# indygreg/python-zstandard

Hardware: NVIDIA H100
Metric: uncompressed GB/s (compress+decompress) (higher is better)
Workload: dtype u8

## Files before the change

### python_zstandard_b200/csrc/zb_entropy.cuh

```cuda
#pragma once

#define ZB_ENT_WS_BYTES   256
#define ZB_ENT_WS_STRIDE  (ZB_ENT_WS_BYTES + 16)
#define ZB_ENT_SKEW(b)    ((((b) + 15u) & ~15u) | 16u)
#define ZB_ENT_DEF_LL     512
#define ZB_ENT_DEF_OF     (ZB_ENT_DEF_LL + 2 * 64)
#define ZB_ENT_DEF_ML     (ZB_ENT_DEF_OF + 2 * 32)
#define ZB_ENT_HEAD_BYTES (ZB_ENT_DEF_ML + 2 * 64)
#define ZB_ENT_POOL_BYTES(W) ((((227 * 1024 - ZB_ENT_HEAD_BYTES) / (W))) & ~15)
#define ZB_ENT_SMEM(W)    ((W) * ZB_ENT_POOL_BYTES(W) + ZB_ENT_HEAD_BYTES)

enum : u32 { ZB_SRC_NONE = 0, ZB_SRC_PREDEF = 1, ZB_SRC_RLE = 2, ZB_SRC_NCOUNT = 3, ZB_SRC_DICT = 4 };
struct ZbTabSrc { u32 kind; u32 sym; const u8* p; u32 n; };

enum : u32 { ZB_BD_FIRST = 1, ZB_BD_FSE_VALID = 2, ZB_BD_SKIP = 4 };
struct ZbBlkDesc {
    u64 hdr_off;
    u64 seq_off, lit_off;
    u32 span;
    u32 frame;
    u32 flags;
    u32 block_max;
    ZbTabSrc dHuf, dLL, dOF, dML;
};
struct ZbBlkExit { u32 rep[3]; u32 err; };

__device__ __forceinline__ u32 zb_warp_incl_scan(u32 v, u32 lane)
{
    #pragma unroll
    for (int d = 1; d < 32; d <<= 1) { u32 y = __shfl_up_sync(0xFFFFFFFFu, v, d); if (lane >= (u32)d) v += y; }
    return v;
}

template <int WORDS, int BITS>
struct ZbPacked {
    static constexpr u32 PER = 32 / BITS, MASK = (1u << BITS) - 1;
    u32 w[WORDS];
    __device__ __forceinline__ void clear() {
        #pragma unroll
        for (int j = 0; j < WORDS; j++) w[j] = 0;
    }
    __device__ __forceinline__ u32 get(u32 i) const {
        u32 const q = i / PER; u32 v = w[0];
        #pragma unroll
        for (int j = 1; j < WORDS; j++) v = q == (u32)j ? w[j] : v;
        return (v >> (BITS * (i - q * PER))) & MASK;
    }
    __device__ __forceinline__ void add(u32 i, u32 v) {
        u32 const q = i / PER, d = v << (BITS * (i - q * PER));
        #pragma unroll
        for (int j = 0; j < WORDS; j++) w[j] += q == (u32)j ? d : 0u;
    }
};
struct ZbRank : ZbPacked<4, 10> {
    __device__ __forceinline__ u32 operator[](u32 wt) const { return get(wt - 1); }
    __device__ __forceinline__ void count(u32 wt) { if (wt) add(wt - 1, 1); }
};

__device__ static u32 zb_huf_weights(u8* ws, const u8* s, u32 n, u32& out_log, u32& out_nsym, ZbRank& rank, ZB_RING_ARG(ring))
{
    u8* const wn = ws;
    u16* const wt = (u16*)(ws + 128);
    u32 nsym, hdr;
    if (n == 0) return 0;
    rank.clear();
    u32 total = 0;
    auto put = [&](u32 i, u32 w) { wn[i >> 1] |= (u8)(w << ((i & 1) * 4)); };
    auto clear_nibbles = [&] { for (int i = 0; i < 32; i++) ((u32*)wn)[i] = 0; };
    if (s[0] >= 128) {
        nsym = (u32)s[0] - 127; hdr = (nsym + 1) / 2;
        if (hdr + 1 > n) return 0;
        clear_nibbles();
        for (u32 i = 0; i < nsym; i++) {
            u32 b = s[1 + i / 2], w = (i & 1) ? (b & 15) : (b >> 4);
            if (w > 12) return 0;
            put(i, w); rank.count(w); total += (1u << w) >> 1;
        }
    } else {
        hdr = s[0];
        if (hdr + 1 > n) return 0;
        short* const norm = (short*)wn; u32 max_sym = 15, log;
        u32 const used = zb_read_ncount(norm, max_sym, log, s + 1, hdr);
        if (used == 0 || log > 6) return 0;
        zb_fse_spread(wt, norm, max_sym, log);
        u32 const size = 1u << log;
        for (u32 u = 0; u < size; u++) {
            u32 const sy = wt[u], x = (u32)(u16)norm[sy]; norm[sy] = (short)(x + 1);
            u32 const nb = log - (u32)zb_hibit(x);
            wt[u] = (u16)(sy | (nb << 4) | (((x << nb) - size) << 8));
        }
        clear_nibbles();
        ZbBitR<4> b;
        if (!b.init(s + 1 + used, hdr - used, ring)) return 0;
        u32 s1 = b.read(log), s2 = b.read(log); b.refill();
        if (b.left() < 0) return 0;
        nsym = 0;
        for (;;) {
            if (nsym + 2 > 255) return 0;
            { u32 c = wt[s1], w = c & 15; if (w > 12) return 0; put(nsym, w); rank.count(w); total += (1u << w) >> 1; nsym++;
              s1 = (c >> 8) + b.read((c >> 4) & 15); b.refill(); }
            if (b.left() < 0) { u32 w = wt[s2] & 15; if (w > 12) return 0; put(nsym, w); rank.count(w); total += (1u << w) >> 1; nsym++; break; }
            if (nsym + 2 > 255) return 0;
            { u32 c = wt[s2], w = c & 15; if (w > 12) return 0; put(nsym, w); rank.count(w); total += (1u << w) >> 1; nsym++;
              s2 = (c >> 8) + b.read((c >> 4) & 15); b.refill(); }
            if (b.left() < 0) { u32 w = wt[s1] & 15; if (w > 12) return 0; put(nsym, w); rank.count(w); total += (1u << w) >> 1; nsym++; break; }
        }
    }
    if (total == 0) return 0;
    u32 const log = (u32)zb_hibit(total) + 1;
    if (log > 12) return 0;
    u32 const rest = (1u << log) - total, hb = (u32)zb_hibit(rest);
    if ((1u << hb) != rest) return 0;
    put(nsym, hb + 1); rank.count(hb + 1); nsym++;
    if (rank[1] < 2 || (rank[1] & 1)) return 0;
    out_log = log; out_nsym = nsym;
    return hdr + 1;
}

#define ZB_HUF_COARSE 8u
struct ZbHufTab { const u16* cells; u32 log, shift, T, base; };
__device__ __forceinline__ void zb_huf_shape(u32 log, ZbRank const& rank, u32& shift, u32& T, u32& base, u32& bytes)
{
    shift = log > ZB_HUF_COARSE ? log - ZB_HUF_COARSE : 0u;
    T = 0;
    #pragma unroll
    for (u32 wt = 1; wt <= 12 - ZB_HUF_COARSE; wt++) T += wt <= shift ? rank[wt] << (wt - 1) : 0u;
    base = (T + 3u) & ~3u;
    bytes = 2u * (base + (1u << (log - shift)));
}
__device__ __forceinline__ ZbHufTab zb_huf_full(const u16* cells, u32 log) { ZbHufTab t; t.cells = cells; t.log = log; t.shift = 0; t.T = 0; t.base = 0; return t; }
#define ZB_HCELL(t, v) ((t).cells[(v) < (t).T ? (v) : (t).base + ((v) >> (t).shift)])

__device__ static void zb_huf_fill(u16* cells, const u8* ws, u32 log, u32 nsym, ZbRank const& rank, u32 shift, u32 base)
{
    ZbPacked<6, 16> next; next.clear();
    {
        u32 p = 0;
        #pragma unroll
        for (u32 wt = 1; wt <= 12; wt++) { next.add(wt - 1, p); p += wt <= log ? (rank[wt] << (wt - 1)) : 0; }
    }
    for (u32 i = 0; i < nsym; i++) {
        u32 const wt = (ws[i >> 1] >> ((i & 1) * 4)) & 15; if (!wt) continue;
        u32 len = 1u << (wt - 1), p = next.get(wt - 1); next.add(wt - 1, len);
        if (wt > shift) { len >>= shift; p = base + (p >> shift); }
        u32 const cell = i | ((log + 1 - wt) << 8);
        if (len >= 4) { u64 const v = cell * 0x0001000100010001ull; u64* q = (u64*)(cells + p); for (u32 k = 0; k < len / 4; k++) q[k] = v; }
        else if (len == 2) *(u32*)(cells + p) = cell * 0x00010001u;
        else cells[p] = (u16)cell;
    }
}

#ifdef ZB_SIMT_EMULATION
__device__ __forceinline__ ZbRank zb_rank_pack(const u32* rank) { ZbRank r; r.clear(); for (u32 wt = 1; wt <= 12; wt++) r.add(wt - 1, rank[wt]); return r; }
__device__ static u32 zb_huf_weights(u8* ws, const u8* s, u32 n, u32& out_log, u32& out_nsym, u32* rank, ZB_RING_ARG(ring))
{
    ZbRank r; u32 const used = zb_huf_weights(ws, s, n, out_log, out_nsym, r, ring);
    rank[0] = used ? out_nsym : 0;
    for (u32 w = 1; w <= 12; w++) { rank[w] = used ? r[w] : 0; rank[0] -= rank[w]; }
    return used;
}
__device__ __forceinline__ void zb_huf_shape(u32 log, const u32* rank, u32& shift, u32& T, u32& base, u32& bytes)
{
    zb_huf_shape(log, zb_rank_pack(rank), shift, T, base, bytes);
}
__device__ static void zb_huf_fill(u16* cells, const u8* ws, u32 log, u32 nsym, const u32* rank, u32 shift, u32 base)
{
    zb_huf_fill(cells, ws, log, nsym, zb_rank_pack(rank), shift, base);
}
#endif

__device__ static bool zb_huf_stream2(u8* out, u32 n_out, const u8* s, u32 n, ZbHufTab const t, u8* ring)
{
    ZbBitR<4> b;
    if (!b.init(s, n, ring)) return false;
    u32 const log = t.log;
    u32 i = 0;
    while (i < n_out && ((uintptr_t)(out + i) & 3)) { u32 v = b.peek(log); u32 c = ZB_HCELL(t, v); out[i++] = (u8)c; b.skip(c >> 8); b.refill(); }
    for (; i + 4 <= n_out; i += 4) {
        u32 v0 = b.peek(log); u32 c0 = ZB_HCELL(t, v0); b.skip(c0 >> 8);
        u32 v1 = b.peek(log); u32 c1 = ZB_HCELL(t, v1); b.skip(c1 >> 8); b.refill();
        u32 v2 = b.peek(log); u32 c2 = ZB_HCELL(t, v2); b.skip(c2 >> 8);
        u32 v3 = b.peek(log); u32 c3 = ZB_HCELL(t, v3); b.skip(c3 >> 8); b.refill();
        *(u32*)(out + i) = (c0 & 255) | ((c1 & 255) << 8) | ((c2 & 255) << 16) | (c3 << 24);
    }
    for (; i < n_out; i++) { u32 v = b.peek(log); u32 c = ZB_HCELL(t, v); out[i] = (u8)c; b.skip(c >> 8); b.refill(); }
    return b.left() == 0;
}

struct ZbHufLane { ZbBitR<4> b; u8* out; u32 left; };

__device__ __forceinline__ void zb_huf_one(ZbHufLane& h, ZbHufTab const& t)
{
    u32 const v = h.b.peek(t.log); u32 const c = ZB_HCELL(t, v); *h.out++ = (u8)c; h.b.skip(c >> 8); h.b.refill(); h.left--;
}
#define ZB_HUF4(h) do { \
        u32 const v0_ = h.b.peek(t.log); u32 const c0_ = ZB_HCELL(t, v0_); h.b.skip(c0_ >> 8); \
        u32 const v1_ = h.b.peek(t.log); u32 const c1_ = ZB_HCELL(t, v1_); h.b.skip(c1_ >> 8); h.b.refill(); \
        u32 const v2_ = h.b.peek(t.log); u32 const c2_ = ZB_HCELL(t, v2_); h.b.skip(c2_ >> 8); \
        u32 const v3_ = h.b.peek(t.log); u32 const c3_ = ZB_HCELL(t, v3_); h.b.skip(c3_ >> 8); h.b.refill(); \
        *(u32*)h.out = (c0_ & 255) | ((c1_ & 255) << 8) | ((c2_ & 255) << 16) | (c3_ << 24); h.out += 4; h.left -= 4; } while (0)

__device__ static bool zb_huf_block(u8* dstl, u32 regen, const u8* p, u32 left, bool single, ZbHufTab const t, ZB_RING_ARG(ring))
{
    if (single) return zb_huf_stream2(dstl, regen, p, left, t, ring);
    if (left < 10) return false;
    u32 const l1 = zb_rd16(p), l2 = zb_rd16(p + 2), l3 = zb_rd16(p + 4), seg = (regen + 3) / 4;
    if (6 + l1 + l2 + l3 > left || seg * 3 > regen) return false;
    u32 const l4 = left - 6 - l1 - l2 - l3;
    ZbHufLane h0, h1, h2, h3;
    u8* const r1 = ring ? ring + 64 : nullptr; u8* const r2 = ring ? ring + 128 : nullptr; u8* const r3 = ring ? ring + 192 : nullptr;
    if (!h0.b.start(p + 6, l1, ring) || !h1.b.start(p + 6 + l1, l2, r1) || !h2.b.start(p + 6 + l1 + l2, l3, r2) || !h3.b.start(p + 6 + l1 + l2 + l3, l4, r3)) return false;
    if (!h0.b.finish() || !h1.b.finish() || !h2.b.finish() || !h3.b.finish()) return false;
    h0.out = dstl; h1.out = dstl + seg; h2.out = dstl + 2 * seg; h3.out = dstl + 3 * seg;
    h0.left = h1.left = h2.left = seg; h3.left = regen - 3 * seg;
    while (h0.left && ((uintptr_t)h0.out & 3)) zb_huf_one(h0, t);
    while (h1.left && ((uintptr_t)h1.out & 3)) zb_huf_one(h1, t);
    while (h2.left && ((uintptr_t)h2.out & 3)) zb_huf_one(h2, t);
    while (h3.left && ((uintptr_t)h3.out & 3)) zb_huf_one(h3, t);
    while (h0.left >= 4 && h1.left >= 4 && h2.left >= 4 && h3.left >= 4) { ZB_HUF4(h0); ZB_HUF4(h1); ZB_HUF4(h2); ZB_HUF4(h3); }
    while (h0.left >= 4) ZB_HUF4(h0);
    while (h1.left >= 4) ZB_HUF4(h1);
    while (h2.left >= 4) ZB_HUF4(h2);
    while (h3.left >= 4) ZB_HUF4(h3);
    while (h0.left) zb_huf_one(h0, t);
    while (h1.left) zb_huf_one(h1, t);
    while (h2.left) zb_huf_one(h2, t);
    while (h3.left) zb_huf_one(h3, t);
    return h0.b.left() == 0 && h1.b.left() == 0 && h2.b.left() == 0 && h3.b.left() == 0;
}

__device__ static int zb_seq_desc(ZbTabSrc& d, u32 mode, u32 max_sym_kind, u32 max_log, const u8* ip, u32 avail,
                                  bool repeat_ok, short* norm, u32& log, u32& max_sym, u32& need)
{
    int used = 0;
    if (mode == 0) { d.kind = ZB_SRC_PREDEF; }
    else if (mode == 1) { if (avail == 0 || ip[0] > max_sym_kind) return -1; d.kind = ZB_SRC_RLE; d.sym = ip[0]; used = 1; }
    else if (mode == 2) { d.kind = ZB_SRC_NCOUNT; d.p = ip; d.n = avail; }
    else if (!repeat_ok || d.kind == ZB_SRC_NONE) return -1;
    need = 0; log = 0; max_sym = max_sym_kind;
    if (d.kind == ZB_SRC_NCOUNT) {
        u32 const u = zb_read_ncount(norm, max_sym, log, d.p, d.n);
        if (u == 0 || log > max_log) return -1;
        if (mode == 2) { used = (int)u; d.n = u; }
        need = 2u << log;
    } else if (d.kind == ZB_SRC_RLE) need = 2;
    return used;
}

template <class F> __device__ __forceinline__ void zb_cta_for(u32 n, F f)
{
#ifdef __CUDA_ARCH__
    for (u32 i = threadIdx.x; i < n; i += blockDim.x) f(i);
#else
    if (threadIdx.x == 0) for (u32 i = 0; i < n; i++) f(i);
#endif
}

__device__ __forceinline__ void zb_cta_cells16(u8* dst, const ZbFseCell* src, u32 log)
{
    zb_cta_for(1u << log, [&](u32 i) { u32 const c = src[i]; ((u16*)dst)[i] = ZB_CELL16(ZB_CELL_SYM(c), (ZB_CELL_NEXT(c) + (1u << log)) >> ZB_CELL_NB(c)); });
}

template <int W>
__device__ __forceinline__ u32 zb_ent_head(u8* smem, ZbDictDev const& dict)
{
    u32* const lutLL = (u32*)smem; u32* const lutML = lutLL + 36;
    zb_cta_for(36, [&](u32 i) { lutLL[i] = c_LL_base[i] | ((u32)c_LL_bits[i] << 24); });
    zb_cta_for(53, [&](u32 i) { lutML[i] = c_ML_base[i] | ((u32)c_ML_bits[i] << 24); });
    zb_cta_cells16(smem + ZB_ENT_DEF_LL, g_defLL, 6);
    zb_cta_cells16(smem + ZB_ENT_DEF_OF, g_defOF, 5);
    zb_cta_cells16(smem + ZB_ENT_DEF_ML, g_defML, 6);
    u32 head = ZB_ENT_HEAD_BYTES;
    if (dict.has_entropy) {
        zb_cta_cells16(smem + head, dict.ll, dict.ll_log); head += 2u << dict.ll_log;
        zb_cta_cells16(smem + head, dict.of, dict.of_log); head += 2u << dict.of_log;
        zb_cta_cells16(smem + head, dict.ml, dict.ml_log); head += 2u << dict.ml_log;
    }
    __syncthreads();
    return ((ZB_ENT_SMEM(W) - head) / W) & ~15u;
}

#ifdef ZB_PHASE_TIMERS
__device__ unsigned long long g_zb_ent_phase[8];
#define ZB_EMARK(k) do { if (lane == 0) { long long const t_ = clock64(); atomicAdd(&g_zb_ent_phase[k], (unsigned long long)(t_ - t_ph)); t_ph = t_; } } while (0)
#elif defined(ZB_DEBUG_BLOCKS)
#define ZB_EMARK(k) do { if (err && !(t_ph & 1)) { printf("[emark %d] lane %u err %u\n", k, lane, err); t_ph |= 1; } } while (0)
#else
#define ZB_EMARK(k) do { (void)t_ph; } while (0)
#endif

template <bool SYMREP>
__device__ __forceinline__ u32 zb_seq_block(const u8* smem, u8* q, u8* ws, ZbDictDev const& dict,
                                            ZbTabSrc const& dLL, ZbTabSrc const& dOF, ZbTabSrc const& dML,
                                            u32 msLL, u32 msOF, u32 msML, u32 logLL, u32 logOF, u32 logML,
                                            const u8* ip, const u8* bend, u32 nseq, ZbSeq* sq, u32 n_lit, u64 room, u64 hist,
                                            u32& rep0, u32& rep1, u32& rep2, u32& lit_used, u32& produced, long long& t_ph)
{
    const u32* const lutLL = (const u32*)smem; const u32* const lutML = lutLL + 36;
    short* const normLL = (short*)ws; short* const normOF = normLL + 36; short* const normML = normOF + 32;
    u32 const dct_ll = ZB_ENT_HEAD_BYTES, dct_of = dct_ll + (2u << dict.ll_log), dct_ml = dct_of + (2u << dict.of_log);
    ZbTab tLL, tOF, tML;
    auto setup = [&](const ZbTabSrc& d, short* norm, u32 ms, u32 lg, int kind, u32 dct, u32 dlog, u32 def, u32 deflog, ZbTab& t) {
        if (d.kind == ZB_SRC_NCOUNT) { zb_build_fse((u16*)q, norm, ms, lg, kind); t.off = (u32)(q - smem); t.log = lg; q += 2u << lg; }
        else if (d.kind == ZB_SRC_RLE) { *(u16*)q = ZB_CELL16(d.sym, 1u); t.off = (u32)(q - smem); t.log = 0; q += 2; }
        else if (d.kind == ZB_SRC_DICT) { t.off = dct; t.log = dlog; }
        else { t.off = def; t.log = deflog; }
    };
    setup(dLL, normLL, msLL, logLL, K_LL, dct_ll, dict.ll_log, ZB_ENT_DEF_LL, 6, tLL);
    setup(dOF, normOF, msOF, logOF, K_OF, dct_of, dict.of_log, ZB_ENT_DEF_OF, 5, tOF);
    setup(dML, normML, msML, logML, K_ML, dct_ml, dict.ml_log, ZB_ENT_DEF_ML, 6, tML);
#ifdef ZB_PHASE_TIMERS
    { u32 const lane = threadIdx.x & 31; ZB_EMARK(7); }
#endif

    ZbBitR<8> b;
    if (!b.init(ip, (u32)(bend - ip), ws)) return ZB_E_CORRUPTION;
    u32 sLL = b.read(tLL.log); u32 sOF = b.read(tOF.log); b.refill(); u32 sML = b.read(tML.log);
    const u8* const TL = smem + tLL.off; const u8* const TO = smem + tOF.off; const u8* const TM = smem + tML.off;
    u32 const kL = 31 - tLL.log, kO = 31 - tOF.log, kM = 31 - tML.log;
    u32 err = ZB_OK;
    for (u32 i = 0; i < nseq; i++) {
        u32 const cl = *(const u16*)(TL + 2 * sLL), co = *(const u16*)(TO + 2 * sOF), cm = *(const u16*)(TM + 2 * sML);
        b.refill();
        u32 const llc = cl & 63, ofc = co & 63, xl = cl >> 6, xo = co >> 6, xm = cm >> 6;
        u32 const nl = __clz(xl) - kL, nm = __clz(xm) - kM, no = __clz(xo) - kO;
        u32 const eL = lutLL[llc], eM = lutML[cm & 63];
        u32 const llb = eL >> 24, ab = (eM >> 24) + llb;
        u32 const sb = i + 1 < nseq ? nl + nm + no : 0;
        bool const slow = (int)(ofc + ab + sb) > b.avail;
        u32 const ob = b.read(ofc);
        u32 ll = eL & 0xFFFFFFu, ml = eM & 0xFFFFFFu, off;
        if (ofc > 1) {
            off = (1u << ofc) - 3 + ob;
            if (SYMREP && (off & 0x80000000u)) { err = ZB_E_CORRUPTION; break; }
            rep2 = rep1; rep1 = rep0; rep0 = off;
        } else {
            u32 const ll0 = (llc == 0);
            if (ofc == 0) {
                if (ll0) { off = rep1; rep1 = rep0; rep0 = off; } else off = rep0;
            } else {
                u32 const idx = 1 + ll0 + ob;
                u32 const r0m = SYMREP && (rep0 & 0x80000000u) ? rep0 + 1 : rep0 - 1;
                u32 tmp = idx == 1 ? rep1 : (idx == 2 ? rep2 : r0m);
                if (SYMREP && tmp == 0) { err = ZB_E_CORRUPTION; break; }
                if (tmp == 0) tmp = 0xFFFFFFFFu;
                if (idx != 1) rep2 = rep1;
                rep1 = rep0; rep0 = off = tmp;
            }
        }
        if (slow) b.refill();
        {
            u32 const both = b.read(ab);
            ml += both >> llb; ll += both & ((1u << llb) - 1);
        }
        if (slow) b.refill();
        {
            u32 const v = b.read(sb);
            sLL = (xl << nl) - (1u << tLL.log) + (v >> (nm + no));
            sML = (xm << nm) - (1u << tML.log) + ((v >> no) & ((1u << nm) - 1));
            sOF = (xo << no) - (1u << tOF.log) + (v & ((1u << no) - 1));
        }
        sq[i] = make_uint4(lit_used, produced, ml, off);
        if ((u64)produced + ll + ml > room) { err = ZB_E_DSTSIZE_TOO_SMALL; break; }
        if (ll > n_lit - lit_used) { err = ZB_E_CORRUPTION; break; }
        lit_used += ll; produced += ll;
        if ((u64)off > hist + produced) { err = ZB_E_CORRUPTION; break; }
        produced += ml;
    }
    if (!err && b.left() != 0) err = ZB_E_CORRUPTION;
    return err;
}

template <int ZB_ENT_WARPS>
__global__ void __launch_bounds__(ZB_ENT_WARPS * 32)
zb_entropy_decode(const u8* __restrict__ src, const ZbSegment* __restrict__ segs, u32 n_frames,
                  const ZbFramePlace* __restrict__ place, const u64* __restrict__ dst_sizes,
                  ZbBlock* __restrict__ blocks, ZbSeq* __restrict__ seqs, u8* __restrict__ lits,
                  u32* __restrict__ work_counter, ZbDictDev dict, u32* status, u64* __restrict__ out_sizes,
                  u32* __restrict__ ck_expect, u32 take)
{
    ZB_DYN_SMEM(zb_smem);
    u32 const lane = threadIdx.x & 31, warp = threadIdx.x >> 5;
    u32 const pool_bytes = zb_ent_head<ZB_ENT_WARPS>(zb_smem, dict);
    u8* const pool = zb_smem + ZB_ENT_SMEM(ZB_ENT_WARPS) - (ZB_ENT_WARPS - warp) * pool_bytes;
    u8* const ws = pool + lane * ZB_ENT_WS_STRIDE;
    u8* const tabs = pool + 32 * ZB_ENT_WS_STRIDE;
    u32 const TAB_BYTES = pool_bytes - 32 * ZB_ENT_WS_STRIDE;

    for (;;) {
        u32 base = 0;
        if (lane == 0) base = atomicAdd(work_counter, take);
        base = __shfl_sync(0xFFFFFFFFu, base, 0);
        if (base >= n_frames) return;
        u32 const f = base + lane;
        bool done = lane >= take || !(f < n_frames) || status[f] != ZB_OK;

        const u8* s = src; u64 n = 0; ZbHdr h; ZbFramePlace pl; u32 err = ZB_OK;
        u64 cap = 0, out_pos = 0, blk_i = 0, seq_i = 0, lit_i = 0, pos = 0; u32 block_max = 0;
        u32 rep0 = 1, rep1 = 4, rep2 = 8;
        ZbTabSrc dHuf = {ZB_SRC_NONE, 0, nullptr, 0}, dLL = dHuf, dOF = dHuf, dML = dHuf;
        bool fse_valid = false;
        if (!done) {
            s = src + segs[f].offset; n = segs[f].length;
            zb_skip_skippable(s, n);
            zb_parse_header(s, n, h);
            pl = place[f]; cap = pl.dst_cap; blk_i = pl.blk_off; seq_i = pl.seq_off; lit_i = pl.lit_off; pos = h.hdr_size;
            block_max = h.window < ZB_BLOCK_MAX ? (u32)h.window : ZB_BLOCK_MAX;
            if (dict.has_entropy) {
                dHuf.kind = dLL.kind = dOF.kind = dML.kind = ZB_SRC_DICT; fse_valid = true;
                rep0 = dict.rep[0]; rep1 = dict.rep[1]; rep2 = dict.rep[2];
            }
            if (h.dict_id && dict.dict_id && h.dict_id != dict.dict_id) { err = ZB_E_DICT_WRONG; done = true; }
        }
        u64 const hist_extra = dict.content_size;

        long long t_ph = clock64() & ~1ll;
        while (__any_sync(0xFFFFFFFFu, !done)) {
            ZB_EMARK(0);
            ZbBlock B; B.kind = 0; B.regen = 0; B.n_seq = 0; B.n_lit = 0; B.lit_kind = 0; B.lit_byte = 0; B.src_pos = 0; B.seq_pos = seq_i; B.out_pos = out_pos;
            bool comp = false, last = false;
            u32 bsize = 0; const u8* bs = nullptr; const u8* bend = nullptr; const u8* ip = nullptr;
            ZbLitHdr L; L.type = 0; L.regen = 0; L.hdr = 0; L.csize = 0; L.single = 0;
            if (!done) {
                do {
                    if (pos + 3 > n) { err = ZB_E_SRCSIZE_WRONG; break; }
                    u32 const bh = zb_rd24(s + pos); pos += 3;
                    last = bh & 1; u32 const type = (bh >> 1) & 3; bsize = bh >> 3; B.kind = type;
                    if (type == 3) { err = ZB_E_CORRUPTION; break; }
                    if (type == ZB_BLK_RLE) {
                        if (pos + 1 > n) { err = ZB_E_SRCSIZE_WRONG; break; }
                        if (bsize > block_max) { err = ZB_E_CORRUPTION; break; }
                        if (bsize > cap - out_pos) { err = ZB_E_DSTSIZE_TOO_SMALL; break; }
                        B.src_pos = (u64)(s + pos - src); B.regen = bsize; B.lit_byte = s[pos]; pos += 1;
                    } else if (type == ZB_BLK_RAW) {
                        if (pos + bsize > n) { err = ZB_E_SRCSIZE_WRONG; break; }
                        if (bsize > block_max) { err = ZB_E_CORRUPTION; break; }
                        if (bsize > cap - out_pos) { err = ZB_E_DSTSIZE_TOO_SMALL; break; }
                        B.src_pos = (u64)(s + pos - src); B.regen = bsize; pos += bsize;
                    } else {
                        if (pos + bsize > n || bsize > block_max) { err = ZB_E_SRCSIZE_WRONG; break; }
                        bs = s + pos; bend = bs + bsize;
                        err = zb_parse_lit_header(bs, bsize, L);
                        if (err) break;
                        if (L.regen > block_max) { err = ZB_E_CORRUPTION; break; }
                        B.n_lit = L.regen; comp = true;
                    }
                } while (0);
                if (err) { done = true; comp = false; }
            }
            ZB_EMARK(1);
            bool wantH = false; u32 hlog = 0, hns = 0; ZbRank rank; const u8* hp = nullptr; u32 hleft = 0;
            if (comp) {
                do {
                    if (L.type == 0) {
                        if (L.hdr + L.regen > bsize) { err = ZB_E_CORRUPTION; break; }
                        B.lit_kind = ZB_LIT_RAW; B.src_pos = (u64)(bs + L.hdr - src); ip = bs + L.hdr + L.regen;
                    } else if (L.type == 1) {
                        if (L.hdr + 1 > bsize) { err = ZB_E_CORRUPTION; break; }
                        B.lit_kind = ZB_LIT_RLE; B.lit_byte = bs[L.hdr]; ip = bs + L.hdr + 1;
                    } else {
                        if (L.type == 3 && dHuf.kind == ZB_SRC_NONE) { err = ZB_E_DICT_CORRUPTED; break; }
                        if (!L.single && L.regen < 6) { err = ZB_E_LITERALS_HEADER_WRONG; break; }
                        if (L.csize + L.hdr > bsize || L.regen == 0) { err = ZB_E_CORRUPTION; break; }
                        hp = bs + L.hdr; hleft = L.csize;
                        if (L.type == 2) { dHuf.kind = ZB_SRC_NCOUNT; dHuf.p = hp; dHuf.n = hleft; }
                        if (dHuf.kind == ZB_SRC_NCOUNT) {
                            u32 const used = zb_huf_weights(ws, dHuf.p, dHuf.n, hlog, hns, rank, tabs + lane * 80);
                            if (used == 0 || (L.type == 2 && used >= hleft)) { err = ZB_E_CORRUPTION; break; }
                            if (L.type == 2) { hp += used; hleft -= used; dHuf.n = used; }
                            wantH = true;
                        }
                        B.lit_kind = ZB_LIT_SCRATCH; B.src_pos = lit_i; ip = bs + L.hdr + L.csize;
                    }
                } while (0);
                if (err) { done = true; comp = false; wantH = false; }
            }
            if (comp && B.lit_kind == ZB_LIT_SCRATCH && dHuf.kind == ZB_SRC_DICT) {
                if (!zb_huf_block(lits + lit_i, L.regen, hp, hleft, L.single, zb_huf_full(dict.huf, dict.huf_log), ws)) { err = ZB_E_CORRUPTION; done = true; comp = false; }
            }
            ZB_EMARK(2);
            {
                bool pending = wantH;
                u32 hshift = 0, hT = 0, hbase = 0, hbytes = 0;
                if (wantH) zb_huf_shape(hlog, rank, hshift, hT, hbase, hbytes);
                while (__any_sync(0xFFFFFFFFu, pending)) {
                    u32 const need = pending ? hbytes : 0;
                    u32 const incl = zb_warp_incl_scan((need + 15) & ~15u, lane);
                    if (pending && incl <= TAB_BYTES) {
                        u16* cells = (u16*)(tabs + incl - ((need + 15) & ~15u));
                        zb_huf_fill(cells, ws, hlog, hns, rank, hshift, hbase);
                        ZB_EMARK(6);
                        ZbHufTab t; t.cells = cells; t.log = hlog; t.shift = hshift; t.T = hT; t.base = hbase;
                        if (!zb_huf_block(lits + lit_i, L.regen, hp, hleft, L.single, t, ws)) { err = ZB_E_CORRUPTION; done = true; comp = false; }
                        pending = false;
                    }
                    __syncwarp();
                }
            }
            ZB_EMARK(3);
            if (comp && B.lit_kind == ZB_LIT_SCRATCH) lit_i += (L.regen + 15) & ~15u;
            u32 nseq = 0, logLL = 0, logOF = 0, logML = 0, msLL = 0, msOF = 0, msML = 0, needS = 0;
            short* const normLL = (short*)ws; short* const normOF = normLL + 36; short* const normML = normOF + 32;
            if (comp) {
                do {
                    if (ip >= bend) { err = ZB_E_SRCSIZE_WRONG; break; }
                    nseq = *ip++;
                    if (nseq > 0x7F) {
                        if (nseq == 0xFF) { if (ip + 2 > bend) { err = ZB_E_SRCSIZE_WRONG; break; } nseq = zb_rd16(ip) + 0x7F00; ip += 2; }
                        else { if (ip >= bend) { err = ZB_E_SRCSIZE_WRONG; break; } nseq = ((nseq - 0x80) << 8) + *ip++; }
                    }
                    B.n_seq = nseq;
                    if (nseq == 0) { if (ip != bend) err = ZB_E_CORRUPTION; break; }
                    if (ip + 1 > bend) { err = ZB_E_SRCSIZE_WRONG; break; }
                    u32 const modes = *ip++;
                    if (modes & 3) { err = ZB_E_CORRUPTION; break; }
                    u32 nd; int r;
                    r = zb_seq_desc(dLL, modes >> 6, 35, 9, ip, (u32)(bend - ip), fse_valid, normLL, logLL, msLL, nd);
                    if (r < 0) { err = ZB_E_CORRUPTION; break; } ip += r; needS += nd;
                    r = zb_seq_desc(dOF, (modes >> 4) & 3, 31, 8, ip, (u32)(bend - ip), fse_valid, normOF, logOF, msOF, nd);
                    if (r < 0) { err = ZB_E_CORRUPTION; break; } ip += r; needS += nd;
                    r = zb_seq_desc(dML, (modes >> 2) & 3, 52, 9, ip, (u32)(bend - ip), fse_valid, normML, logML, msML, nd);
                    if (r < 0) { err = ZB_E_CORRUPTION; break; } ip += r; needS += nd;
                    fse_valid = true;
                } while (0);
                if (err) { done = true; comp = false; nseq = 0; }
            }
            ZB_EMARK(4);
            u32 lit_used = 0, produced = 0;
            {
                bool pending = comp && nseq > 0;
                while (__any_sync(0xFFFFFFFFu, pending)) {
                    u32 const need = pending ? ZB_ENT_SKEW(needS) : 0;
                    u32 const incl = zb_warp_incl_scan(need, lane);
                    if (pending && incl <= TAB_BYTES) {
                        err = zb_seq_block<false>(zb_smem, tabs + incl - need, ws, dict, dLL, dOF, dML, msLL, msOF, msML, logLL, logOF, logML,
                                                   ip, bend, nseq, seqs + seq_i, L.regen, cap - out_pos, out_pos + hist_extra,
                                                   rep0, rep1, rep2, lit_used, produced, t_ph);
                        if (err) { done = true; comp = false; }
                        pending = false;
                    }
                    __syncwarp();
                }
            }
            ZB_EMARK(5);
            if (!done) {
                if (comp) {
                    seqs[seq_i + nseq] = make_uint4(lit_used, produced, 0, 0);
                    seq_i += nseq + 1;
                    u32 const tail = L.regen - lit_used;
                    if ((u64)produced + tail > cap - out_pos) err = ZB_E_DSTSIZE_TOO_SMALL;
                    B.regen = produced + tail;
                    if (!err && B.regen > block_max) err = ZB_E_CORRUPTION;
                    pos += bsize;
                }
                if (!err) {
                    blocks[blk_i++] = B;
                    out_pos += B.regen;
                    if (last) {
                        if (h.content_size != ZB_CONTENT_UNKNOWN && out_pos != h.content_size) err = ZB_E_CORRUPTION;
                        else if (h.checksum && pos + 4 > n) err = ZB_E_CHECKSUM_WRONG;
                        else {
                            if (h.checksum) ck_expect[f] = zb_rd32(s + pos);
                            if (dst_sizes && out_pos != cap) err = ZB_E_SIZE_MISMATCH;
                        }
                        done = true;
                    }
                }
                if (err) done = true;
            }
        }
        if (lane < take && f < n_frames && status[f] == ZB_OK) {
            if (err) { status[f] = err; out_sizes[f] = err == ZB_E_SIZE_MISMATCH ? out_pos : 0; } else out_sizes[f] = out_pos;
        } else if (lane < take && f < n_frames) out_sizes[f] = 0;
    }
}

template <int ZB_ENT_WARPS>
__global__ void __launch_bounds__(ZB_ENT_WARPS * 32)
zb_entropy_blocks(const u8* __restrict__ src, const ZbBlkDesc* __restrict__ bdesc, u32 n_blocks,
                  ZbBlock* __restrict__ blocks, ZbSeq* __restrict__ seqs, u8* __restrict__ lits,
                  u32* __restrict__ work_counter, ZbDictDev dict, u32* status, ZbBlkExit* __restrict__ bexit, u32 take)
{
    ZB_DYN_SMEM(zb_smem);
    u32 const lane = threadIdx.x & 31, warp = threadIdx.x >> 5;
    u32 const pool_bytes = zb_ent_head<ZB_ENT_WARPS>(zb_smem, dict);
    u8* const pool = zb_smem + ZB_ENT_SMEM(ZB_ENT_WARPS) - (ZB_ENT_WARPS - warp) * pool_bytes;
    u8* const ws = pool + lane * ZB_ENT_WS_BYTES;
    u8* const tabs = pool + 32 * ZB_ENT_WS_BYTES;
    u32 const TAB_BYTES = pool_bytes - 32 * ZB_ENT_WS_BYTES;

    for (;;) {
        u32 base = 0;
        if (lane == 0) base = atomicAdd(work_counter, take);
        base = __shfl_sync(0xFFFFFFFFu, base, 0);
        if (base >= n_blocks) return;
        u32 const bi = base + lane;
        ZbBlkDesc D; D.frame = 0; D.flags = 0;
        if (lane < take && bi < n_blocks) D = bdesc[bi];
        bool done = lane >= take || !(bi < n_blocks) || (D.flags & ZB_BD_SKIP) || status[D.frame] != ZB_OK;

        const u8* s = src; u64 n = 0; u32 err = ZB_OK;
        u64 const cap = ~0ull >> 1; u64 out_pos = 0, blk_i = bi, seq_i = 0, lit_i = 0, pos = 0; u32 block_max = 0;
        u32 rep0 = 1, rep1 = 4, rep2 = 8;
        ZbTabSrc dHuf = {ZB_SRC_NONE, 0, nullptr, 0}, dLL = dHuf, dOF = dHuf, dML = dHuf;
        bool fse_valid = false;
        if (!done) {
            s = src + D.hdr_off; n = D.span; seq_i = D.seq_off; lit_i = D.lit_off; block_max = D.block_max;
            dHuf = D.dHuf; dLL = D.dLL; dOF = D.dOF; dML = D.dML; fse_valid = (D.flags & ZB_BD_FSE_VALID) != 0;
            if (D.flags & ZB_BD_FIRST) { if (dict.has_entropy) { rep0 = dict.rep[0]; rep1 = dict.rep[1]; rep2 = dict.rep[2]; } }
            else { rep0 = 0x80000000u; rep1 = 0xA0000000u; rep2 = 0xC0000000u; }
        }
        u64 const hist_extra = 1ull << 40;

        long long t_ph = clock64() & ~1ll;
        while (__any_sync(0xFFFFFFFFu, !done)) {
            ZB_EMARK(0);
            ZbBlock B; B.kind = 0; B.regen = 0; B.n_seq = 0; B.n_lit = 0; B.lit_kind = 0; B.lit_byte = 0; B.src_pos = 0; B.seq_pos = seq_i; B.out_pos = out_pos;
            bool comp = false, last = false;
            u32 bsize = 0; const u8* bs = nullptr; const u8* bend = nullptr; const u8* ip = nullptr;
            ZbLitHdr L; L.type = 0; L.regen = 0; L.hdr = 0; L.csize = 0; L.single = 0;
            if (!done) {
                do {
                    if (pos + 3 > n) { err = ZB_E_SRCSIZE_WRONG; break; }
                    u32 const bh = zb_rd24(s + pos); pos += 3;
                    last = bh & 1; u32 const type = (bh >> 1) & 3; bsize = bh >> 3; B.kind = type;
                    if (type == 3) { err = ZB_E_CORRUPTION; break; }
                    if (type == ZB_BLK_RLE) {
                        if (pos + 1 > n) { err = ZB_E_SRCSIZE_WRONG; break; }
                        if (bsize > block_max) { err = ZB_E_CORRUPTION; break; }
                        if (bsize > cap - out_pos) { err = ZB_E_DSTSIZE_TOO_SMALL; break; }
                        B.src_pos = (u64)(s + pos - src); B.regen = bsize; B.lit_byte = s[pos]; pos += 1;
                    } else if (type == ZB_BLK_RAW) {
                        if (pos + bsize > n) { err = ZB_E_SRCSIZE_WRONG; break; }
                        if (bsize > block_max) { err = ZB_E_CORRUPTION; break; }
                        if (bsize > cap - out_pos) { err = ZB_E_DSTSIZE_TOO_SMALL; break; }
                        B.src_pos = (u64)(s + pos - src); B.regen = bsize; pos += bsize;
                    } else {
                        if (pos + bsize > n || bsize > block_max) { err = ZB_E_SRCSIZE_WRONG; break; }
                        bs = s + pos; bend = bs + bsize;
                        err = zb_parse_lit_header(bs, bsize, L);
                        if (err) break;
                        if (L.regen > block_max) { err = ZB_E_CORRUPTION; break; }
                        B.n_lit = L.regen; comp = true;
                    }
                } while (0);
                if (err) { done = true; comp = false; }
            }
            ZB_EMARK(1);
            bool wantH = false; u32 hlog = 0, hns = 0; ZbRank rank; const u8* hp = nullptr; u32 hleft = 0;
            if (comp) {
                do {
                    if (L.type == 0) {
                        if (L.hdr + L.regen > bsize) { err = ZB_E_CORRUPTION; break; }
                        B.lit_kind = ZB_LIT_RAW; B.src_pos = (u64)(bs + L.hdr - src); ip = bs + L.hdr + L.regen;
                    } else if (L.type == 1) {
                        if (L.hdr + 1 > bsize) { err = ZB_E_CORRUPTION; break; }
                        B.lit_kind = ZB_LIT_RLE; B.lit_byte = bs[L.hdr]; ip = bs + L.hdr + 1;
                    } else {
                        if (L.type == 3 && dHuf.kind == ZB_SRC_NONE) { err = ZB_E_DICT_CORRUPTED; break; }
                        if (!L.single && L.regen < 6) { err = ZB_E_LITERALS_HEADER_WRONG; break; }
                        if (L.csize + L.hdr > bsize || L.regen == 0) { err = ZB_E_CORRUPTION; break; }
                        hp = bs + L.hdr; hleft = L.csize;
                        if (L.type == 2) { dHuf.kind = ZB_SRC_NCOUNT; dHuf.p = hp; dHuf.n = hleft; }
                        if (dHuf.kind == ZB_SRC_NCOUNT) {
                            u32 const used = zb_huf_weights(ws, dHuf.p, dHuf.n, hlog, hns, rank, tabs + lane * 64);
                            if (used == 0 || (L.type == 2 && used >= hleft)) { err = ZB_E_CORRUPTION; break; }
                            if (L.type == 2) { hp += used; hleft -= used; dHuf.n = used; }
                            wantH = true;
                        }
                        B.lit_kind = ZB_LIT_SCRATCH; B.src_pos = lit_i; ip = bs + L.hdr + L.csize;
                    }
                } while (0);
                if (err) { done = true; comp = false; wantH = false; }
            }
            if (comp && B.lit_kind == ZB_LIT_SCRATCH && dHuf.kind == ZB_SRC_DICT) {
                if (!zb_huf_block(lits + lit_i, L.regen, hp, hleft, L.single, zb_huf_full(dict.huf, dict.huf_log), ws)) { err = ZB_E_CORRUPTION; done = true; comp = false; }
            }
            ZB_EMARK(2);
            {
                bool pending = wantH;
                u32 hshift = 0, hT = 0, hbase = 0, hbytes = 0;
                if (wantH) zb_huf_shape(hlog, rank, hshift, hT, hbase, hbytes);
                while (__any_sync(0xFFFFFFFFu, pending)) {
                    u32 const need = pending ? hbytes : 0;
                    u32 const incl = zb_warp_incl_scan((need + 15) & ~15u, lane);
                    if (pending && incl <= TAB_BYTES) {
                        u16* cells = (u16*)(tabs + incl - ((need + 15) & ~15u));
                        zb_huf_fill(cells, ws, hlog, hns, rank, hshift, hbase);
                        ZB_EMARK(6);
                        ZbHufTab t; t.cells = cells; t.log = hlog; t.shift = hshift; t.T = hT; t.base = hbase;
                        if (!zb_huf_block(lits + lit_i, L.regen, hp, hleft, L.single, t, ws)) { err = ZB_E_CORRUPTION; done = true; comp = false; }
                        pending = false;
                    }
                    __syncwarp();
                }
            }
            ZB_EMARK(3);
            if (comp && B.lit_kind == ZB_LIT_SCRATCH) lit_i += (L.regen + 15) & ~15u;
            u32 nseq = 0, logLL = 0, logOF = 0, logML = 0, msLL = 0, msOF = 0, msML = 0, needS = 0;
            short* const normLL = (short*)ws; short* const normOF = normLL + 36; short* const normML = normOF + 32;
            if (comp) {
                do {
                    if (ip >= bend) { err = ZB_E_SRCSIZE_WRONG; break; }
                    nseq = *ip++;
                    if (nseq > 0x7F) {
                        if (nseq == 0xFF) { if (ip + 2 > bend) { err = ZB_E_SRCSIZE_WRONG; break; } nseq = zb_rd16(ip) + 0x7F00; ip += 2; }
                        else { if (ip >= bend) { err = ZB_E_SRCSIZE_WRONG; break; } nseq = ((nseq - 0x80) << 8) + *ip++; }
                    }
                    B.n_seq = nseq;
                    if (nseq == 0) { if (ip != bend) err = ZB_E_CORRUPTION; break; }
                    if (ip + 1 > bend) { err = ZB_E_SRCSIZE_WRONG; break; }
                    u32 const modes = *ip++;
                    if (modes & 3) { err = ZB_E_CORRUPTION; break; }
                    u32 nd; int r;
                    r = zb_seq_desc(dLL, modes >> 6, 35, 9, ip, (u32)(bend - ip), fse_valid, normLL, logLL, msLL, nd);
                    if (r < 0) { err = ZB_E_CORRUPTION; break; } ip += r; needS += nd;
                    r = zb_seq_desc(dOF, (modes >> 4) & 3, 31, 8, ip, (u32)(bend - ip), fse_valid, normOF, logOF, msOF, nd);
                    if (r < 0) { err = ZB_E_CORRUPTION; break; } ip += r; needS += nd;
                    r = zb_seq_desc(dML, (modes >> 2) & 3, 52, 9, ip, (u32)(bend - ip), fse_valid, normML, logML, msML, nd);
                    if (r < 0) { err = ZB_E_CORRUPTION; break; } ip += r; needS += nd;
                    fse_valid = true;
                } while (0);
                if (err) { done = true; comp = false; nseq = 0; }
            }
            ZB_EMARK(4);
            u32 lit_used = 0, produced = 0;
            {
                bool pending = comp && nseq > 0;
                while (__any_sync(0xFFFFFFFFu, pending)) {
                    u32 const need = pending ? ((needS + 15) & ~15u) : 0;
                    u32 const incl = zb_warp_incl_scan(need, lane);
                    if (pending && incl <= TAB_BYTES) {
                        err = zb_seq_block<true>(zb_smem, tabs + incl - need, ws, dict, dLL, dOF, dML, msLL, msOF, msML, logLL, logOF, logML,
                                                   ip, bend, nseq, seqs + seq_i, L.regen, cap - out_pos, out_pos + hist_extra,
                                                   rep0, rep1, rep2, lit_used, produced, t_ph);
                        if (err) { done = true; comp = false; }
                        pending = false;
                    }
                    __syncwarp();
                }
            }
            ZB_EMARK(5);
            if (!done) {
                if (comp) {
                    seqs[seq_i + nseq] = make_uint4(lit_used, produced, 0, 0);
                    seq_i += nseq + 1;
                    u32 const tail = L.regen - lit_used;
                    if ((u64)produced + tail > cap - out_pos) err = ZB_E_DSTSIZE_TOO_SMALL;
                    B.regen = produced + tail;
                    if (!err && B.regen > block_max) err = ZB_E_CORRUPTION;
                    pos += bsize;
                }
                if (!err) blocks[blk_i] = B;
                done = true;
            }
        }
        if (lane < take && bi < n_blocks && !(D.flags & ZB_BD_SKIP)) {
            ZbBlkExit X; X.rep[0] = rep0; X.rep[1] = rep1; X.rep[2] = rep2; X.err = err;
            bexit[bi] = X;
#ifdef ZB_DEBUG_BLOCKS
            if (err) printf("[entropy_blocks] block %u frame %u err %u flags %u span %u | huf k%u n%u | LL k%u n%u s%u | OF k%u n%u s%u | ML k%u n%u s%u | hdr %02x %02x %02x | LLp-src %lld\n", bi, D.frame, err, D.flags, D.span,
                            D.dHuf.kind, D.dHuf.n, D.dLL.kind, D.dLL.n, D.dLL.sym, D.dOF.kind, D.dOF.n, D.dOF.sym, D.dML.kind, D.dML.n, D.dML.sym,
                            src[D.hdr_off], src[D.hdr_off + 1], src[D.hdr_off + 2], D.dLL.p ? (long long)(D.dLL.p - src) : -1ll);
#endif
            if (err) atomicCAS(&status[D.frame], (u32)ZB_OK, err);
        }
    }
}
```

Before: 147.9.

## Stage decoded sequences in shared memory and write them out warp-cooperatively

The per-lane sequence decode loop now writes each decoded sequence to a per-lane shared-memory staging ring of eight entries instead of storing it directly to global memory. Every eight sequences the warp synchronizes, and lanes cooperatively copy the staged entries to global memory, with eight lanes covering each source lane's batch, so that scattered 16-byte global stores become coalesced 128-byte bursts. The function is now called by all lanes, with a go flag, so that warp-collective shuffles work. In exchange it adds warp synchronization every eight sequences, which forces divergent lanes to wait on one another, and uses part of the workspace as staging with a stride that differs between the two call sites.

```diff
diff --git a/python_zstandard_b200/csrc/zb_entropy.cuh b/python_zstandard_b200/csrc/zb_entropy.cuh
--- a/python_zstandard_b200/csrc/zb_entropy.cuh
+++ b/python_zstandard_b200/csrc/zb_entropy.cuh
@@ -290,84 +290,109 @@
 #endif
 
 template <bool SYMREP>
-__device__ __forceinline__ u32 zb_seq_block(const u8* smem, u8* q, u8* ws, ZbDictDev const& dict,
+__device__ __forceinline__ u32 zb_seq_block(bool go, const u8* smem, u8* q, u8* ws, u32 ws_stride, ZbDictDev const& dict,
                                             ZbTabSrc const& dLL, ZbTabSrc const& dOF, ZbTabSrc const& dML,
                                             u32 msLL, u32 msOF, u32 msML, u32 logLL, u32 logOF, u32 logML,
                                             const u8* ip, const u8* bend, u32 nseq, ZbSeq* sq, u32 n_lit, u64 room, u64 hist,
                                             u32& rep0, u32& rep1, u32& rep2, u32& lit_used, u32& produced, long long& t_ph)
 {
+    u32 const lane = threadIdx.x & 31;
     const u32* const lutLL = (const u32*)smem; const u32* const lutML = lutLL + 36;
     short* const normLL = (short*)ws; short* const normOF = normLL + 36; short* const normML = normOF + 32;
     u32 const dct_ll = ZB_ENT_HEAD_BYTES, dct_of = dct_ll + (2u << dict.ll_log), dct_ml = dct_of + (2u << dict.of_log);
-    ZbTab tLL, tOF, tML;
+    ZbTab tLL = {0, 0}, tOF = tLL, tML = tLL;
     auto setup = [&](const ZbTabSrc& d, short* norm, u32 ms, u32 lg, int kind, u32 dct, u32 dlog, u32 def, u32 deflog, ZbTab& t) {
         if (d.kind == ZB_SRC_NCOUNT) { zb_build_fse((u16*)q, norm, ms, lg, kind); t.off = (u32)(q - smem); t.log = lg; q += 2u << lg; }
         else if (d.kind == ZB_SRC_RLE) { *(u16*)q = ZB_CELL16(d.sym, 1u); t.off = (u32)(q - smem); t.log = 0; q += 2; }
         else if (d.kind == ZB_SRC_DICT) { t.off = dct; t.log = dlog; }
         else { t.off = def; t.log = deflog; }
     };
-    setup(dLL, normLL, msLL, logLL, K_LL, dct_ll, dict.ll_log, ZB_ENT_DEF_LL, 6, tLL);
-    setup(dOF, normOF, msOF, logOF, K_OF, dct_of, dict.of_log, ZB_ENT_DEF_OF, 5, tOF);
-    setup(dML, normML, msML, logML, K_ML, dct_ml, dict.ml_log, ZB_ENT_DEF_ML, 6, tML);
+    u32 err = ZB_OK;
+    ZbBitR<8> b;
+    u32 sLL = 0, sOF = 0, sML = 0;
+    if (go) {
+        setup(dLL, normLL, msLL, logLL, K_LL, dct_ll, dict.ll_log, ZB_ENT_DEF_LL, 6, tLL);
+        setup(dOF, normOF, msOF, logOF, K_OF, dct_of, dict.of_log, ZB_ENT_DEF_OF, 5, tOF);
+        setup(dML, normML, msML, logML, K_ML, dct_ml, dict.ml_log, ZB_ENT_DEF_ML, 6, tML);
 #ifdef ZB_PHASE_TIMERS
-    { u32 const lane = threadIdx.x & 31; ZB_EMARK(7); }
+        ZB_EMARK(7);
 #endif
-
-    ZbBitR<8> b;
-    if (!b.init(ip, (u32)(bend - ip), ws)) return ZB_E_CORRUPTION;
-    u32 sLL = b.read(tLL.log); u32 sOF = b.read(tOF.log); b.refill(); u32 sML = b.read(tML.log);
+        if (!b.init(ip, (u32)(bend - ip), ws)) err = ZB_E_CORRUPTION;
+        else { sLL = b.read(tLL.log); sOF = b.read(tOF.log); b.refill(); sML = b.read(tML.log); }
+    }
     const u8* const TL = smem + tLL.off; const u8* const TO = smem + tOF.off; const u8* const TM = smem + tML.off;
     u32 const kL = 31 - tLL.log, kO = 31 - tOF.log, kM = 31 - tML.log;
-    u32 err = ZB_OK;
-    for (u32 i = 0; i < nseq; i++) {
-        u32 const cl = *(const u16*)(TL + 2 * sLL), co = *(const u16*)(TO + 2 * sOF), cm = *(const u16*)(TM + 2 * sML);
-        b.refill();
-        u32 const llc = cl & 63, ofc = co & 63, xl = cl >> 6, xo = co >> 6, xm = cm >> 6;
-        u32 const nl = __clz(xl) - kL, nm = __clz(xm) - kM, no = __clz(xo) - kO;
-        u32 const eL = lutLL[llc], eM = lutML[cm & 63];
-        u32 const llb = eL >> 24, ab = (eM >> 24) + llb;
-        u32 const sb = i + 1 < nseq ? nl + nm + no : 0;
-        bool const slow = (int)(ofc + ab + sb) > b.avail;
-        u32 const ob = b.read(ofc);
-        u32 ll = eL & 0xFFFFFFu, ml = eM & 0xFFFFFFu, off;
-        if (ofc > 1) {
-            off = (1u << ofc) - 3 + ob;
-            if (SYMREP && (off & 0x80000000u)) { err = ZB_E_CORRUPTION; break; }
-            rep2 = rep1; rep1 = rep0; rep0 = off;
-        } else {
-            u32 const ll0 = (llc == 0);
-            if (ofc == 0) {
-                if (ll0) { off = rep1; rep1 = rep0; rep0 = off; } else off = rep0;
-            } else {
-                u32 const idx = 1 + ll0 + ob;
-                u32 const r0m = SYMREP && (rep0 & 0x80000000u) ? rep0 + 1 : rep0 - 1;
-                u32 tmp = idx == 1 ? rep1 : (idx == 2 ? rep2 : r0m);
-                if (SYMREP && tmp == 0) { err = ZB_E_CORRUPTION; break; }
-                if (tmp == 0) tmp = 0xFFFFFFFFu;
-                if (idx != 1) rep2 = rep1;
-                rep1 = rep0; rep0 = off = tmp;
-            }
-        }
-        if (slow) b.refill();
-        {
-            u32 const both = b.read(ab);
-            ml += both >> llb; ll += both & ((1u << llb) - 1);
-        }
-        if (slow) b.refill();
-        {
-            u32 const v = b.read(sb);
-            sLL = (xl << nl) - (1u << tLL.log) + (v >> (nm + no));
-            sML = (xm << nm) - (1u << tML.log) + ((v >> no) & ((1u << nm) - 1));
-            sOF = (xo << no) - (1u << tOF.log) + (v & ((1u << no) - 1));
-        }
-        sq[i] = make_uint4(lit_used, produced, ml, off);
-        if ((u64)produced + ll + ml > room) { err = ZB_E_DSTSIZE_TOO_SMALL; break; }
-        if (ll > n_lit - lit_used) { err = ZB_E_CORRUPTION; break; }
-        lit_used += ll; produced += ll;
-        if ((u64)off > hist + produced) { err = ZB_E_CORRUPTION; break; }
-        produced += ml;
-    }
-    if (!err && b.left() != 0) err = ZB_E_CORRUPTION;
+    u8* const stage = ws + 128;
+    bool run = go && !err;
+    u32 i = 0;
+    for (u32 i0 = 0; __any_sync(0xFFFFFFFFu, run && i0 < nseq); i0 += 8) {
+        bool const ran = run && i0 < nseq;
+        if (ran) {
+            while (i < nseq) {
+                u32 const cl = *(const u16*)(TL + 2 * sLL), co = *(const u16*)(TO + 2 * sOF), cm = *(const u16*)(TM + 2 * sML);
+                b.refill();
+                u32 const llc = cl & 63, ofc = co & 63, xl = cl >> 6, xo = co >> 6, xm = cm >> 6;
+                u32 const nl = __clz(xl) - kL, nm = __clz(xm) - kM, no = __clz(xo) - kO;
+                u32 const eL = lutLL[llc], eM = lutML[cm & 63];
+                u32 const llb = eL >> 24, ab = (eM >> 24) + llb;
+                u32 const sb = i + 1 < nseq ? nl + nm + no : 0;
+                bool const slow = (int)(ofc + ab + sb) > b.avail;
+                u32 const ob = b.read(ofc);
+                u32 ll = eL & 0xFFFFFFu, ml = eM & 0xFFFFFFu, off;
+                if (ofc > 1) {
+                    off = (1u << ofc) - 3 + ob;
+                    if (SYMREP && (off & 0x80000000u)) { err = ZB_E_CORRUPTION; break; }
+                    rep2 = rep1; rep1 = rep0; rep0 = off;
+                } else {
+                    u32 const ll0 = (llc == 0);
+                    if (ofc == 0) {
+                        if (ll0) { off = rep1; rep1 = rep0; rep0 = off; } else off = rep0;
+                    } else {
+                        u32 const idx = 1 + ll0 + ob;
+                        u32 const r0m = SYMREP && (rep0 & 0x80000000u) ? rep0 + 1 : rep0 - 1;
+                        u32 tmp = idx == 1 ? rep1 : (idx == 2 ? rep2 : r0m);
+                        if (SYMREP && tmp == 0) { err = ZB_E_CORRUPTION; break; }
+                        if (tmp == 0) tmp = 0xFFFFFFFFu;
+                        if (idx != 1) rep2 = rep1;
+                        rep1 = rep0; rep0 = off = tmp;
+                    }
+                }
+                if (slow) b.refill();
+                {
+                    u32 const both = b.read(ab);
+                    ml += both >> llb; ll += both & ((1u << llb) - 1);
+                }
+                if (slow) b.refill();
+                {
+                    u32 const v = b.read(sb);
+                    sLL = (xl << nl) - (1u << tLL.log) + (v >> (nm + no));
+                    sML = (xm << nm) - (1u << tML.log) + ((v >> no) & ((1u << nm) - 1));
+                    sOF = (xo << no) - (1u << tOF.log) + (v & ((1u << no) - 1));
+                }
+                *(ZbSeq*)(stage + 16 * (i & 7)) = make_uint4(lit_used, produced, ml, off);
+                i++;
+                if ((u64)produced + ll + ml > room) { err = ZB_E_DSTSIZE_TOO_SMALL; break; }
+                if (ll > n_lit - lit_used) { err = ZB_E_CORRUPTION; break; }
+                lit_used += ll; produced += ll;
+                if ((u64)off > hist + produced) { err = ZB_E_CORRUPTION; break; }
+                produced += ml;
+                if (!(i & 7)) break;
+            }
+            run = !err;
+        }
+        __syncwarp();
+        u64 const mine = (u64)(uintptr_t)(sq + i0) | (ran ? i - i0 : 0u);
+        u8* const stage0 = stage - lane * ws_stride;
+        u32 const r = lane & 7;
+        #pragma unroll 1
+        for (u32 j = 0; j < 8; j++) {
+            u32 const o = 4 * j + (lane >> 3);
+            u64 const p = __shfl_sync(0xFFFFFFFFu, mine, o);
+            if (r < (u32)(p & 15)) ((ZbSeq*)(uintptr_t)(p & ~15ull))[r] = *(const ZbSeq*)(stage0 + o * ws_stride + 16 * r);
+        }
+        __syncwarp();
+    }
+    if (go && !err && b.left() != 0) err = ZB_E_CORRUPTION;
     return err;
 }
 
@@ -532,14 +557,15 @@
                 while (__any_sync(0xFFFFFFFFu, pending)) {
                     u32 const need = pending ? ZB_ENT_SKEW(needS) : 0;
                     u32 const incl = zb_warp_incl_scan(need, lane);
-                    if (pending && incl <= TAB_BYTES) {
-                        err = zb_seq_block<false>(zb_smem, tabs + incl - need, ws, dict, dLL, dOF, dML, msLL, msOF, msML, logLL, logOF, logML,
-                                                   ip, bend, nseq, seqs + seq_i, L.regen, cap - out_pos, out_pos + hist_extra,
-                                                   rep0, rep1, rep2, lit_used, produced, t_ph);
+                    bool const go = pending && incl <= TAB_BYTES;
+                    u32 const e = zb_seq_block<false>(go, zb_smem, tabs + incl - need, ws, ZB_ENT_WS_STRIDE, dict, dLL, dOF, dML,
+                                                      msLL, msOF, msML, logLL, logOF, logML, ip, bend, nseq, seqs + seq_i, L.regen,
+                                                      cap - out_pos, out_pos + hist_extra, rep0, rep1, rep2, lit_used, produced, t_ph);
+                    if (go) {
+                        err = e;
                         if (err) { done = true; comp = false; }
                         pending = false;
                     }
-                    __syncwarp();
                 }
             }
             ZB_EMARK(5);
@@ -730,14 +756,15 @@
                 while (__any_sync(0xFFFFFFFFu, pending)) {
                     u32 const need = pending ? ((needS + 15) & ~15u) : 0;
                     u32 const incl = zb_warp_incl_scan(need, lane);
-                    if (pending && incl <= TAB_BYTES) {
-                        err = zb_seq_block<true>(zb_smem, tabs + incl - need, ws, dict, dLL, dOF, dML, msLL, msOF, msML, logLL, logOF, logML,
-                                                   ip, bend, nseq, seqs + seq_i, L.regen, cap - out_pos, out_pos + hist_extra,
-                                                   rep0, rep1, rep2, lit_used, produced, t_ph);
+                    bool const go = pending && incl <= TAB_BYTES;
+                    u32 const e = zb_seq_block<true>(go, zb_smem, tabs + incl - need, ws, ZB_ENT_WS_BYTES, dict, dLL, dOF, dML,
+                                                     msLL, msOF, msML, logLL, logOF, logML, ip, bend, nseq, seqs + seq_i, L.regen,
+                                                     cap - out_pos, out_pos + hist_extra, rep0, rep1, rep2, lit_used, produced, t_ph);
+                    if (go) {
+                        err = e;
                         if (err) { done = true; comp = false; }
                         pending = false;
                     }
-                    __syncwarp();
                 }
             }
             ZB_EMARK(5);
```

Result: faster. 161.1, median of 6 (+8.9%).
